# open-rmf/rmf_crowdsim

Measured on AMD Instinct MI355X. Metric: agent-steps/sec at 1M agents, dt=0.05 s; % HBM roofline on Zanlungo kernel, higher is better.
Workload: dtype f32

## Files before the change

### rmf_crowdsim_amd/csrc/crowdstep_hip.hip

```cpp

#include <hip/hip_runtime.h>
#include <chrono>

#include <algorithm>
#include <cmath>
#include <cstdint>
#include <cstdio>
#include <array>
#include <cmath>
#include <cstring>
#include <functional>
#include <map>
#include <string>
#include <thread>
#include <tuple>
#include <vector>

#include "crowdstep.h"
#include "crowdstep_state.h"

#define CS_INVALID_CELL 0xFFFFFFFFu
#define CS_MAX_GROUPS 1048575u
#define CS_SPAWN_OCCUPANCY_RADIUS 0.4
#define CS_ID_LIMIT 0x7FFFFFFFull
// ... 163 lines not shown
      if (const char* w = getenv("CS_FIRST_DEVICE_ID")) {
        const uint64_t d = std::min<uint64_t>((uint64_t)strtoull(w, nullptr, 10), e->id_limit - 2u);
        e->dev_base = e->next_id = (d & ~1ull) | (e->ext_base & 1u);
      }
    }
    const uint32_t nid = (uint32_t)e->next_id;
    if (ok) hipMemcpy(&e->ctr->next_id, &nid, sizeof nid, hipMemcpyHostToDevice);
  }
  if (!ok || e->upload_sinks() != 0 ||
      e->reserve(cfg && cfg->capacity_hint ? cfg->capacity_hint : 1024) != 0) {
    return create_failed(e, "device allocation failed: " + e->error);
  }
  return e;
}

const char* cs_last_error(const cs_engine* e) { return e ? e->error.c_str() : g_create_error.c_str(); }
const char* cs_backend_name(const cs_engine* e) { return e ? e->backend.c_str() : ""; }

uint32_t cs_register_zanlungo(cs_engine* e, const cs_zanlungo_params* p) {
  e->lp_params.push_back(*p);
  e->lp_kinds.push_back(1u);
  e->lp_callbacks.emplace_back();
  return (uint32_t)e->lp_kinds.size() - 1;
}
uint32_t cs_register_no_local_plan(cs_engine* e) {
  cs_zanlungo_params z;
  std::memset(&z, 0, sizeof z);
  z.agent_mass = 1.0;
  z.force_distance = 1.0;
  e->lp_params.push_back(z);
  e->lp_kinds.push_back(0u);
  e->lp_callbacks.emplace_back();
  return (uint32_t)e->lp_kinds.size() - 1;
}
uint32_t cs_register_lp_callback(cs_engine* e, cs_lp_batch_fn fn, void* user) {
  if (!fn) {
    e->error = "cs_register_lp_callback: the planner's function is null";
    return UINT32_MAX;
  }
  cs_zanlungo_params z;
  std::memset(&z, 0, sizeof z);
  z.agent_mass = 1.0;
  z.force_distance = 1.0;
  e->lp_params.push_back(z);
  e->lp_kinds.push_back(2u);
  cs_engine::LpCallback cb;
  cb.fn = fn;
  cb.user = user;
  e->lp_callbacks.push_back(cb);
  return (uint32_t)e->lp_kinds.size() - 1;
}
uint32_t cs_register_hlp(cs_engine* e, const cs_hlp_desc* d) {
  if (d->kind == CS_HLP_ROUTE) {
    if (!d->route_plan || !(d->route_scale > 0.0) || !(d->route_arrive >= 0.0)) {
      e->error = "route planner: route_plan, route_scale > 0 and route_arrive >= 0 are required";
      return UINT32_MAX;
    }
  }
  e->hlps.push_back(*d);
  return (uint32_t)e->hlps.size() - 1;
}

int cs_add_agents(cs_engine* e, const double* xy, size_t n, uint32_t hlp, uint32_t lp,
                  double eyesight, uint64_t* out_ids) {
  hipSetDevice(e->device);
  if (hlp >= e->hlps.size() || lp >= e->lp_kinds.size()) {
    e->error = "unknown planner handle";
    return 2;
  }
  if (e->plain_groups.find(std::make_tuple(hlp, lp, eyesight)) == e->plain_groups.end())
    if (int rc = e->room_for_group(0)) return rc;
  uint32_t g = e->make_group(hlp, lp, eyesight, -1);
  return e->add_agents(xy, n, g, UINT32_MAX, out_ids);
}

int cs_remove_agent(cs_engine* e, uint64_t id) {
  hipSetDevice(e->device);
  e->halo_invalidate();
  for (size_t k = 0; k < e->limbo.size(); ++k)
    if (e->limbo[k].id == id) {
      const HostGroup& g = e->groups[e->limbo[k].group];
      const cs_hlp_desc& p = e->hlps[g.hlp];
      if (p.kind == CS_HLP_CALLBACK && p.remove_agent) p.remove_agent(p.user, id);
      e->limbo.erase(e->limbo.begin() + (long)k);
      cs_event ev;
      ev.kind = CS_EVENT_DESTROYED;
      ev.source_sink = UINT32_MAX;
      ev.id = id;
      ev.x = ev.y = 0;
      if (e->record_events) e->events.push_back(ev);
      return 0;
    }
  if (int rc = e->refresh_counts()) return rc;
  uint32_t found[2] = {0xFFFFFFFFu, 0u};
  uint64_t dev = 0;
  if (e->dev_id(id, &dev) && dev < 0xFFFFFFFFull && e->n_slots) {
    if (!e->find_dev && hipMalloc(&e->find_dev, 2 * sizeof(uint32_t)) != hipSuccess) {
      e->error = "HIP error while removing an agent";
      return 90;
    }
    bool ok = hipMemcpyAsync(e->find_dev, found, sizeof found, hipMemcpyHostToDevice, e->stream) == hipSuccess;
    hipLaunchKernelGGL(k_remove_by_id, dim3((e->n_slots + 255u) / 256u), dim3(256), 0, e->stream, e->gdev, e->buf[e->cur],
                       e->n_slots, e->ctr, e->gdev.tile, (e->tile && e->ghosts_present) ? 1u : 0u, (uint32_t)dev,
                       e->find_dev);
    ok = ok && hipMemcpyAsync(found, e->find_dev, sizeof found, hipMemcpyDeviceToHost, e->stream) == hipSuccess &&
         hipStreamSynchronize(e->stream) == hipSuccess;
    if (!ok) {
      e->error = "HIP error while removing an agent";
      return 90;
    }
  }
  if (found[0] == 0xFFFFFFFFu) {
    e->error = "unknown agent id";
    return 2;
  }
  const HostGroup& g = e->groups[meta_group(e->gdev, found[1])];
  const cs_hlp_desc& p = e->hlps[g.hlp];
  if (p.kind == CS_HLP_CALLBACK && p.remove_agent) p.remove_agent(p.user, id);
  e->sorted = false;
  e->hist_valid = false;
  e->occ_valid = false;
  e->halo_invalidate();
  e->n_alive_host -= 1;
  cs_event ev;
  ev.kind = CS_EVENT_DESTROYED;
  ev.source_sink = g.sink >= 0 ? (uint32_t)g.sink : UINT32_MAX;
  ev.id = id;
  ev.x = ev.y = 0;
  if (e->record_events) e->events.push_back(ev);
  return 0;
}

size_t cs_source_sink_slots(cs_engine* e) { return e->sinks.size(); }
uint64_t cs_device_bytes(cs_engine* e) { return e->device_bytes(); }

uint64_t cs_kernel_stat(cs_engine* e, uint32_t which) {
  hipSetDevice(e->device);
  if (which == CS_STAT_EXCHANGES_AHEAD) return e->n_exchanges_ahead;
  if (which == CS_STAT_EXCHANGES_AHEAD_USED) return e->n_exchanges_ahead_used;
  if (which == CS_STAT_STEPS_ON_KEPT_WINDOWS) return e->n_steps_on_kept_windows;
  if (which == CS_STAT_RENUMBERINGS) return e->n_renumberings;
  if (which == CS_STAT_RENUMBER_NS) return e->renumber_ns;
  if (which == CS_STAT_WINDOWS_LISTED) {
    uint64_t n = 0;
    return e->windows_listed(&n) ? 0 : n;
  }
  Counters c;
  if (e->read_counters(&c)) return 0;
  switch (which) {
    case CS_STAT_WINDOWS_OFF_LDS: return c.n_win_off_lds;
    case CS_STAT_WINDOWS_CHUNKED: return c.n_win_chunked;
#ifdef CS_TILE_TRIPS
    case 100: case 101: case 102: case 103: case 104: case 105: case 106: case 107: case 108: case 109: case 110: case 111:
    case 112: case 113: case 114: case 115: case 116:
      return c.dbg[which - 100];
#endif
    default: return 0;
  }
}

uint32_t cs_add_source_sink(cs_engine* e, const cs_source_sink_desc* d) {
  if (d->n_waypoints == 0) {
    e->error = "a source-sink needs at least one waypoint";
    return UINT32_MAX;
  }
  hipSetDevice(e->device);
  if (e->room_for_group(d->n_waypoints)) return UINT32_MAX;
  HostSink s;
  s.d = *d;
  s.waypoints.assign(d->waypoints_xy, d->waypoints_xy + 2 * d->n_waypoints);
  s.d.waypoints_xy = nullptr;
  uint32_t handle = (uint32_t)e->sinks.size();
  if (e->tile && d->hlp < e->hlps.size() && e->hlps[d->hlp].kind == CS_HLP_ROUTE) {
    s.spawn_route = e->route_lookup(d->hlp, d->source_x, d->source_y, s.waypoints[0], s.waypoints[1]);
    if (!s.spawn_route) {
      e->error = "route planner found no route for this source-sink (tile engines plan at registration)";
      return UINT32_MAX;
    }
  }
  s.group = e->make_group(d->hlp, d->lp, d->agent_eyesight_range, (int32_t)handle);
  e->sinks.push_back(s);
  e->sinks_dirty = true;
  return handle;
}

void cs_remove_source_sink(cs_engine* e, uint32_t handle) {
  if (handle < e->sinks.size() && e->sinks[handle].alive) {
    e->sinks[handle].alive = false;
    e->sinks_dirty = true;
  }
}

int cs_step(cs_engine* e, double dt_seconds, cs_step_report* report) {
  hipSetDevice(e->device);
  const int rc = e->step(dt_seconds, report);
  if (rc == 0) e->steps_done += 1;
  return rc;
}

int cs_snapshot_request(cs_engine* e) {
  hipSetDevice(e->device);
  return e->snapshot_request();
}

int cs_snapshot_acquire(cs_engine* e, int wait, const cs_snapshot_record** out, size_t* n,
                        uint64_t* step_index) {
  hipSetDevice(e->device);
  return e->snapshot_acquire(wait, out, n, step_index);
}

int cs_synchronize(cs_engine* e) {
  hipSetDevice(e->device);
  if (int rc = e->refresh_counts()) return rc;
  Counters c;
  if (int rc = e->read_counters(&c)) return rc;
  e->prof_collect();
  if (c.n_out_of_bounds) {
    e->poisoned = true;
    e->error = "Index out of bounds";
    return 1;
  }
  return 0;
}

size_t cs_agent_count(cs_engine* e) {
  hipSetDevice(e->device);
  e->refresh_counts();
  if (e->tile && e->ghosts_present && e->n_slots) {
    uint32_t owned = 0;
    bool ok = e->find_dev || hipMalloc(&e->find_dev, 2 * sizeof(uint32_t)) == hipSuccess;
    ok = ok && hipMemsetAsync(e->find_dev, 0, sizeof(uint32_t), e->stream) == hipSuccess;
    if (ok)
      hipLaunchKernelGGL(k_tile_count_owned, dim3((e->n_slots + 255u) / 256u), dim3(256), 0, e->stream, e->gdev,
                         e->buf[e->cur], e->n_slots, e->ctr, e->find_dev);
    ok = ok && hipMemcpyAsync(&owned, e->find_dev, sizeof owned, hipMemcpyDeviceToHost, e->stream) == hipSuccess &&
         hipStreamSynchronize(e->stream) == hipSuccess;
    if (ok) return (size_t)owned + e->limbo.size();
    e->error = "HIP error while counting the agents of a tile that holds ghosts";
  }
  return (size_t)e->n_alive_host + e->limbo.size();
}

size_t cs_read_agents(cs_engine* e, cs_agent_view* out, size_t cap) {
  hipSetDevice(e->device);
  if (e->refresh_counts() != 0) return 0;
  cs_engine::HostState h;
  if (e->download(&h) != 0) return 0;
  const bool owned_only = e->tile && e->ghosts_present;
  uint32_t in_use = e->n_slots;
  if (owned_only) {
    Counters c;
    if (e->read_counters(&c) != 0) return 0;
    in_use = std::min(in_use, c.n_pending);
  }
  const GridDev& g = e->gdev;
  std::vector<uint32_t> live;
  for (uint32_t i = 0; i < in_use; ++i) {
    if (h.cell[i] == CS_INVALID_CELL) continue;
    if (owned_only) {
      const uint32_t cx = h.cell[i] / g.nx, cy = h.cell[i] - cx * g.nx;
      if (cx < g.own_x0 || cx >= g.own_x1 || cy < g.own_y0 || cy >= g.own_y1) continue;
    }
    live.push_back(i);
  }
  std::sort(live.begin(), live.end(), [&](uint32_t a, uint32_t b) { return h.id[a] < h.id[b]; });
  size_t n = std::min(cap, live.size());
  for (size_t k = 0; k < n; ++k) {
    uint32_t i = live[k];
    out[k].id = e->ext_id(h.id[i]);
    e->to_global(h.cell[i], h.off[i].x, h.off[i].y, &out[k].x, &out[k].y);
    out[k].vx = h.vel[i].x;
    out[k].vy = h.vel[i].y;
    out[k].next_waypoint = meta_waypoint(e->gdev, h.meta[i]);
    out[k].eyesight_range = e->groups[meta_group(e->gdev, h.meta[i])].eyesight;
  }
  if (!e->limbo.empty()) {
    for (const cs_engine::LimboAgent& l : e->limbo) {
      if (n >= cap) break;
      cs_agent_view v;
      std::memset(&v, 0, sizeof v);
      v.id = l.id;
      v.x = l.x;
      v.y = l.y;
      v.eyesight_range = e->groups[l.group].eyesight;
      out[n++] = v;
    }
    std::sort(out, out + n, [](const cs_agent_view& a, const cs_agent_view& b) { return a.id < b.id; });
  }
  return n;
}

size_t cs_drain_events(cs_engine* e, cs_event* out, size_t cap) {
  size_t n = std::min(cap, e->events.size());
  for (size_t i = 0; i < n; ++i) out[i] = e->events[i];
  e->events.erase(e->events.begin(), e->events.begin() + n);
  return n;
}

void cs_event_recording(cs_engine* e, int on) {
  hipSetDevice(e->device);
  e->refresh_counts();
  e->record_events = on != 0;
  if (!on) e->events.clear();
}

static size_t radius_query(cs_engine* e, double radius, double x, double y, std::vector<uint32_t>* ids,
                           std::vector<float>* d2, size_t cap, bool every_alias) {
// ... 688 lines not shown
```

### rmf_crowdsim_amd/csrc/cs_device_types.hip.inc

```

struct GridDev {
  uint32_t nx;
  uint32_t ny;
  uint32_t ncells;
  float cs;
  float cs_lo;
  float inv_cs;
  uint32_t tile;
  uint32_t own_x0, own_x1, own_y0, own_y1;
  uint32_t org_x, org_y;
  int32_t cs_fix;
  float fix_scale, fix_inv;
  uint32_t grp_bits;
};
__host__ __device__ inline uint32_t meta_group(const GridDev& g, uint32_t meta) { return meta & ((1u << g.grp_bits) - 1u); }
__host__ __device__ inline uint32_t meta_waypoint(const GridDev& g, uint32_t meta) { return meta >> g.grp_bits; }
__host__ __device__ inline uint32_t meta_make(const GridDev& g, uint32_t group, uint32_t waypoint) {
  return group | (waypoint << g.grp_bits);
}

#define FIX_LIM 0x20000000
#define FIX_FAR 0x40000000
__device__ __forceinline__ bool fix_ok(float off, const GridDev& g) {
  return fabsf(off * g.fix_scale) < (float)FIX_LIM;
}
__device__ __forceinline__ int fix_coord(float off, const GridDev& g) {
  return __float2int_rn(off * g.fix_scale);
}
__device__ __forceinline__ void fix_rel(const GridDev& g, float2 oi, float2 oj, int sx, int sy, float& fx,
                                        float& fy) {
  if (fix_ok(oi.x, g) && fix_ok(oi.y, g) && fix_ok(oj.x, g) && fix_ok(oj.y, g) && abs(sx) <= 32 && abs(sy) <= 32) {
    fx = (float)(fix_coord(oj.x, g) - fix_coord(oi.x, g) + sx * g.cs_fix);
    fy = (float)(fix_coord(oj.y, g) - fix_coord(oi.y, g) + sy * g.cs_fix);
  } else {
    fx = ((oj.x + (float)sx * g.cs) - oi.x) * g.fix_scale;
    fy = ((oj.y + (float)sy * g.cs) - oi.y) * g.fix_scale;
  }
}

struct GroupDev {
  float eyesight;
  uint32_t lp_kind;
  float A, D, inv_mass, R;
  uint32_t hlp_kind;
  float hvx, hvy;
  int32_t sink;
  uint32_t hlp;
  float vanish2;
};

struct SelGroupDev {
  uint32_t sink, hlp, lp;
};

struct SinkDev {
  double src_x, src_y;
  uint32_t src_cell;
  uint32_t ghost_cell;
  float src_ox, src_oy;
  float radius_sink;
  uint32_t wp_begin, wp_count;
  uint32_t loop_forever;
  uint32_t group;
  float eyesight;
  uint32_t spawn_route;
};

struct Counters {
  uint32_t n_alive;
  uint32_t n_out_of_bounds;
  uint32_t n_owned;
  uint32_t n_pending;
  uint32_t next_id;
  uint32_t n_spawned;
  uint32_t n_halo_overflow;
  uint32_t n_destroyed;
  uint32_t n_waypoint_hits;
  uint32_t n_tti_zero;
  uint32_t n_nonfinite;
  uint32_t n_clamped;
  uint32_t n_wp_events;
  uint32_t n_halo_late;
  uint32_t n_win_off_lds, n_win_chunked;
  uint32_t n_win_dropped;
  uint32_t n_scan_stalled;
  uint32_t mesh_fail_step;
  uint32_t border_done, border_flag, n_early_stalled;
#ifdef CS_TILE_TRIPS
  uint32_t dbg[17];
#endif
};

struct AgentArrays {
  float2* off;
  float2* vel;
  uint32_t* id;
  uint32_t* cell;
  uint32_t* meta;
  uint32_t* rank;
  uint32_t* route;
};

__device__ __forceinline__ float f_inf() { return __builtin_huge_valf(); }
__device__ __forceinline__ float f_nan() { return __builtin_nanf(""); }

__device__ __forceinline__ float fast_rcp(float x) { return __builtin_amdgcn_rcpf(x); }
__device__ __forceinline__ float fast_sqrt(float x) { return __builtin_amdgcn_sqrtf(x); }
__device__ __forceinline__ float fast_rsq(float x) { return __builtin_amdgcn_rsqf(x); }
__device__ __forceinline__ float fast_exp2(float x) { return __builtin_amdgcn_exp2f(x); }


__device__ __forceinline__ float ttc_select(float t0, float t1) {
  float t = fmaxf(t0, 0.0f);
  t = !(t0 < 0.0f || t0 > 0.0f) ? t1 : t;
  return (t1 > 0.0f) ? t : f_inf();
}

__device__ __noinline__ float ttc_tiny_f32(float rvx, float rvy, float rpx, float rpy, float d2,
                                           float R2, float tscale) {
  rvx *= tscale;
  rvy *= tscale;
  const float a = __builtin_fmaf(rvx, rvx, rvy * rvy);
  const float bh = __builtin_fmaf(rvx, rpx, rvy * rpy);
  const float c = d2 - R2;
  if (a < 1e-30f) {
    if (bh == 0.0f) return f_inf();
    if (c < 0.0f) return 0.0f;
    return bh < 0.0f ? (-c / (2.0f * bh)) * tscale : f_inf();
  }
  const float disc = __builtin_fmaf(bh, bh, -(a * c));
  const float root = fast_sqrt(disc);
  const float ia = fast_rcp(a) * tscale;
  const float t0 = (-bh - root) * ia;
  const float t1 = (-bh + root) * ia;
  return (disc < 0.0f) ? f_inf() : ttc_select(t0, t1);
}

__device__ __forceinline__ float ttc_core_c_f32(float rvx, float rvy, float rpx, float rpy, float c) {
  const float a = __builtin_fmaf(rvx, rvx, rvy * rvy);
  const float bh = __builtin_fmaf(rvx, rpx, rvy * rpy);
  const float disc = __builtin_fmaf(bh, bh, -(a * c));
  const float root = fast_sqrt(disc);
  const float ia = fast_rcp(a);
  const float t0 = (-bh - root) * ia;
  const float t1 = (-bh + root) * ia;
  return ttc_select(t0, t1);
}
__device__ __forceinline__ float ttc_core_f32(float rvx, float rvy, float rpx, float rpy, float d2,
                                              float R2) {
  return ttc_core_c_f32(rvx, rvy, rpx, rpy, d2 - R2);
}

#define TTC_TINY_KEY (0x2B8CBCCCu - 1u)
__device__ __forceinline__ uint32_t ttc_tiny_key(float rvx, float rvy) {
  return __float_as_uint(fmaxf(fabsf(rvx), fabsf(rvy))) - 1u;
}

#define TTC_HUGE_SPEED 0x1p32f
__device__ __forceinline__ bool ttc_huge(float rvx, float rvy) { return fmaxf(fabsf(rvx), fabsf(rvy)) >= TTC_HUGE_SPEED; }

__device__ __forceinline__ float ttc_f32(float rvx, float rvy, float rpx, float rpy, float d2,
                                         float R2) {
  if (__builtin_expect(ttc_tiny_key(rvx, rvy) < TTC_TINY_KEY, 0))
    return ttc_tiny_f32(rvx, rvy, rpx, rpy, d2, R2, 0x1p48f);
  if (__builtin_expect(ttc_huge(rvx, rvy), 0)) return ttc_tiny_f32(rvx, rvy, rpx, rpy, d2, R2, 0x1p-40f);
  return ttc_core_f32(rvx, rvy, rpx, rpy, d2, R2);
}

__device__ __forceinline__ uint32_t ttc_overlap_key(float d2) { return __float_as_uint(d2) - 1u; }
__device__ __forceinline__ float ttc_pair_f32(float rvx, float rvy, float rpx, float rpy, float d2,
                                              float R2) {
  if (__builtin_expect(ttc_overlap_key(d2) < __float_as_uint(R2) || ttc_huge(rvx, rvy), 0))
    return ttc_f32(rvx, rvy, rpx, rpy, d2, R2);
  return ttc_core_c_f32(rvx, rvy, rpx, rpy, d2 - R2);
}

struct ForceCtx {
  float vix, viy, futx, futy, mag, two_R, k_exp;
};

__device__ __forceinline__ ForceCtx make_force_ctx(float vix, float viy, float Ts, const GroupDev& grp, const GridDev& g) {
  ForceCtx c;
  c.vix = vix;
  c.viy = viy;
  c.futx = vix * Ts;
  c.futy = viy * Ts;
  const float T = Ts * g.fix_inv;
  float speed = sqrtf(__builtin_fmaf(vix, vix, viy * viy));
  if (Ts == 0.0f && speed == 0.0f) speed = fmaxf(fabsf(vix), fabsf(viy));
  float mag = 2.0f * grp.A * speed / T;
  c.mag = (mag >= 1e15f) ? 1e15f : mag;
  c.two_R = grp.R * 2.0f * g.fix_scale;
  c.k_exp = 1.44269504088896341f / grp.D * g.fix_inv;
  return c;
}

__device__ __forceinline__ float sight_margin(float ax, float ay, float nr2) {
  return __builtin_fmaf(ax, ax, __builtin_fmaf(ay, ay, nr2));
}

__device__ __forceinline__ bool wave_any(bool p) { return __builtin_amdgcn_ballot_w64(p) != 0ull; }
__device__ __forceinline__ uint32_t in_vgpr(uint32_t x) {
  uint32_t v;
  asm volatile("v_mov_b32 %0, %1" : "=v"(v) : "s"(x));
  return v;
}

#define CS_LDS __attribute__((address_space(3)))
__device__ __forceinline__ uint32_t lds_addr(const void* p) { return (uint32_t)(uintptr_t)(CS_LDS const char*)p; }
typedef int cs_v4i __attribute__((ext_vector_type(4)));
typedef int cs_v2i __attribute__((ext_vector_type(2)));
typedef float cs_v2f __attribute__((ext_vector_type(2)));
__device__ __forceinline__ int4 lds_ld_i4(uint32_t a) {
  const cs_v4i v = *(CS_LDS const cs_v4i*)(uintptr_t)a;
  return make_int4(v.x, v.y, v.z, v.w);
}
__device__ __forceinline__ int2 lds_ld_i2(uint32_t a) {
  const cs_v2i v = *(CS_LDS const cs_v2i*)(uintptr_t)a;
  return make_int2(v.x, v.y);
}
__device__ __forceinline__ float2 lds_ld_f2(uint32_t a) {
  const cs_v2f v = *(CS_LDS const cs_v2f*)(uintptr_t)a;
  return make_float2(v.x, v.y);
}
__device__ __forceinline__ uint32_t lds_ld_u32(uint32_t a) { return *(CS_LDS const uint32_t*)(uintptr_t)a; }
__device__ __forceinline__ uint32_t lds_ld_u16(uint32_t a) { return *(CS_LDS const unsigned short*)(uintptr_t)a; }
__device__ __forceinline__ void lds_st_u16(uint32_t a, uint32_t v) { *(CS_LDS unsigned short*)(uintptr_t)a = (unsigned short)v; }

__device__ __forceinline__ void zanlungo_forward_force(float rpx, float rpy, float d2,
                                                       const ForceCtx& c, float& fx, float& fy) {
  const float dx = c.futx - rpx, dy = c.futy - rpy;
  const float dist = fast_sqrt(__builtin_fmaf(dx, dx, dy * dy));
  float px = rpy, py = -rpx;
  const bool flip = __builtin_fmaf(px, c.vix, py * c.viy) < 0.0f;
  px = flip ? -px : px;
  py = flip ? -py : py;
  const float s = fabsf(__builtin_fmaf(px, dy, -(py * dx)));
  const float inv_n = (s > 0.0f) ? fast_rsq(d2) : f_nan();
  const float scale = c.mag * fast_exp2((c.two_R - dist) * c.k_exp) * inv_n;
  fx = __builtin_fmaf(px, scale, fx);
  fy = __builtin_fmaf(py, scale, fy);
}

#define ZAN_EXP2_ZERO 160.0f

__device__ __forceinline__ bool zanlungo_forward_vanishes(const ForceCtx& c, float Ts, float vanish2) {
  const float fut2 = __builtin_fmaf(c.futx, c.futx, c.futy * c.futy);
  return Ts > 0.0f && Ts < f_inf() && fabsf(c.mag) < f_inf() && fut2 >= vanish2;
}
inline float zanlungo_vanish2(float eyesight, float R, float D, const GridDev& g) {
  const float k_exp = 1.44269504088896341f / D * g.fix_inv;
  const float rs = eyesight * g.fix_scale, two_R = R * 2.0f * g.fix_scale;
  if (!(k_exp >= 0x1p-126f && k_exp < HUGE_VALF && std::fabs(rs) < HUGE_VALF && std::fabs(two_R) < HUGE_VALF))
    return std::nanf("");
  const double b = ((double)std::fabs(rs) + std::max((double)two_R, 0.0) + (double)ZAN_EXP2_ZERO / (double)k_exp) *
                   (1.0 + 0x1p-10);
  const float b2 = std::nextafter((float)(b * b), HUGE_VALF);
  return b2 < HUGE_VALF ? b2 : std::nanf("");
}

struct RouteBookEntry {
  long long sx, sy, gx, gy;
  uint32_t hlp, route1;
};
__host__ __device__ inline long long route_spatial_hash(double v, double res) {
  const double r = round(v / res);
  if (r != r) return 0;
  if (r >= 9.2e18) return 0x7FFFFFFFFFFFFFFFll;
  if (r <= -9.2e18) return (long long)0x8000000000000000ull;
  return (long long)r;
}
__host__ __device__ inline uint32_t route_book_slot(uint32_t hlp, long long sx, long long sy, long long gx, long long gy) {
  unsigned long long h = 0x9E3779B97F4A7C15ull * (unsigned long long)(hlp + 1u);
  h = (h ^ (unsigned long long)sx) * 0xBF58476D1CE4E5B9ull;
  h = (h ^ (unsigned long long)sy) * 0x94D049BB133111EBull;
  h = (h ^ (unsigned long long)gx) * 0xBF58476D1CE4E5B9ull;
  h = (h ^ (unsigned long long)gy) * 0x94D049BB133111EBull;
  return (uint32_t)(h >> 32);
}
__device__ __forceinline__ uint32_t route_book_find(const RouteBookEntry* __restrict__ book, uint32_t mask,
                                                    uint32_t hlp, long long sx, long long sy, long long gx,
                                                    long long gy) {
  if (!book) return 0u;
  uint32_t k = route_book_slot(hlp, sx, sy, gx, gy) & mask;
  for (uint32_t probe = 0; probe <= mask; ++probe) {
    const RouteBookEntry e = book[k];
    if (e.route1 == 0u) return 0u;
    if (e.hlp == hlp && e.sx == sx && e.sy == sy && e.gx == gx && e.gy == gy) return e.route1;
    k = (k + 1u) & mask;
  }
  return 0u;
}

struct StepParams {
  GridDev g;
  float dt;
  uint32_t n;
  uint32_t has_sinks;
  uint32_t n_src_cells;
  uint32_t halo_late_check;
  uint32_t peek_seq;
};

// ... 131 lines not shown
```

### rmf_crowdsim_amd/csrc/cs_kernels_step.hip.inc

```

struct WpEvent {
  uint32_t id, group, next_wp, cell;
  float ox, oy;
  uint32_t slot, pad;
};

struct EpilogueCore {
  AgentArrays out;
  uint32_t* cell_count;
  Counters* ctr;
  const GroupDev* groups;
  const SinkDev* sinks;
  const double* waypoints;
  double grid_off_x, grid_off_y, cell_size;
  uint2* destroyed;
  uint32_t destroyed_cap;
  WpEvent* wp_events;
  uint32_t wp_events_cap;
  const uint32_t* src_cell_start;
  const uint32_t* src_sorted;
  uint32_t* src_occupied;
  const uint2* route_desc;
  const double* route_xy;
  const RouteBookEntry* route_book;
// ... 890 lines not shown
  const bool tile_huge = XF ? (tile_flags & 1u) != 0u : tile_flags != 0u;
  bool lds_ok = tiled_ok;
  if constexpr (XF) {
    if (tiled_ok && (tile_flags & 2u) != 0u) {
      lds_ok = false;
      if (tid == 0) atomicAdd(&E.ctr->n_win_off_lds, 1u);
    }
  }
  for (uint32_t chunk = 0; chunk < n_own; chunk += TILE_THREADS) {
  const OwnIn L = chunk == 0 ? first_own : load_own(chunk);
  const bool active = L.active;
  const int R = row0 + L.own_r;
  const uint32_t i = L.i;
  Own o;
  o.gx = (uint32_t)R;
  o.gy = L.cell - (uint32_t)R * g.nx;
  o.off = L.off;
  o.v = L.v;
  o.id = L.id;
  o.slot = i;
  const uint32_t meta = L.meta;
  const GroupDev grp = L.grp;
  uint32_t route_st = L.route;
  o.u = active ? hlp_velocity(grp, E, g, o.id, pref, i, o.gx, o.gy, o.off, route_st) : make_float2(0.0f, 0.0f);
  float wx = o.u.x, wy = o.u.y;
  if (active && grp.lp_kind == 2u && E.lp_vel) {
    wx = E.lp_vel[i].x;
    wy = E.lp_vel[i].y;
  }
  const bool zan = active && grp.lp_kind == 1u && o.off.x == o.off.x && o.off.y == o.off.y;
  const bool sight_ok = fabsf(grp.eyesight) < f_inf();

  int lx = 1, hx = 0, ly = 1, hy = 0;
  bool use_tile = false;
  if (zan) {
    const float slack = 0.01f * g.cs;
    const bool regular = o.off.x >= -slack && o.off.x <= g.cs + slack && o.off.y >= -slack &&
                         o.off.y <= g.cs + slack;
    if (lds_ok && regular && sight_ok) {
      const float e = grp.eyesight, ics = g.inv_cs;
      const int blx = (int)fminf(fmaxf(floorf((o.off.x - e) * ics - CS_BOUNDS_EPS), -1e9f), 1e9f);
      const int bhx = (int)fminf(fmaxf(floorf((o.off.x + e) * ics + CS_BOUNDS_EPS), -1e9f), 1e9f);
      const int bly = (int)fminf(fmaxf(floorf((o.off.y - e) * ics - CS_BOUNDS_EPS), -1e9f), 1e9f);
      const int bhy = (int)fminf(fmaxf(floorf((o.off.y + e) * ics + CS_BOUNDS_EPS), -1e9f), 1e9f);
      use_tile = (long long)o.gy + bhy < (long long)g.nx;
      lx = max(blx, -cfg.h);
      hx = min(bhx, cfg.h);
      ly = max(bly, -cfg.h);
      hy = min(bhy, cfg.h);
    }
  }
  if (zan && !use_tile) {
    bool tz;
    gather_agent(P, in, cell_start, o, grp, wx, wy, tz);
    if (tz) atomicAdd(&E.ctr->n_tti_zero, 1u);
  }

  if (lds_ok && !TILE_DEBUG(1u)) {
    const bool mine = zan && use_tile;
    if (!mine) {
      lx = 1; hx = 0; ly = 1; hy = 0;
    }
    const float rs = grp.eyesight * g.fix_scale;
    const float nr2 = -(rs * rs);
    const float Rs = grp.R * g.fix_scale;
    const float R2 = Rs * Rs;
    const int own_row = R - r0;
    const int own_col = (int)o.gy - sy0;
    const int2 pi = window_pos(o.off, own_row, own_col);
    const float pix = (float)pi.x;
    auto rel_x = [&](int xj) {
      if constexpr (XF) return __int_as_float(xj) - pix;
      else return (float)(xj - pi.x);
    };
    uint32_t self_slot = 0xFFFFFFFFu;
    if (mine) {
      if (chunk == 0) {
        self_slot = s_self[tid];
      } else {
        const unsigned short* t = s_tab + own_row * W1 + own_col;
        for (uint32_t j = t[0]; j < t[1]; ++j)
          if (s_id[j] == o.id) self_slot = j;
      }
    }
    entry_t* __restrict__ my_list = s_list + tid;
    const uint32_t CAP = cfg.list_cap;
    const uint32_t CAP_ALL = CAP + cfg.spill_rows;
    uint32_t* __restrict__ my_spill =
        cfg.spill + ((size_t)lidx * cfg.spill_rows) * TILE_THREADS + tid;
    bool spilling = false;
    auto entry_at = [&](uint32_t k) -> uint32_t {
      if (k < CAP) return my_list[k * TILE_THREADS];
      return my_spill[(size_t)(k - CAP) * TILE_THREADS];
    };
    uint32_t cnt = 0, n_back = 0;
    unsigned long long fwd = 0;
    unsigned long long fwd2 = 0;
    float T = f_inf();
    bool flushed = false;
    bool self_listed = false;

    auto rel = [&](uint32_t j, float& rpx, float& rpy) {
      const int2 pj = s_pos[j];
      rpx = rel_x(pj.x);
      rpy = (float)(pj.y - pi.y);
    };
    const uint32_t slot_max = S ? S - 1u : 0u;
    auto run_ttc_impl = [&](uint32_t n, uint32_t k0, auto spill_tag) {
      constexpr bool SPILL = decltype(spill_tag)::value;
      uint32_t m_lo = 0, m_hi = 0, m_2 = 0, m_3 = 0;
      for (uint32_t k = k0; __any(k < n); k += 2) {
        const bool v0 = k < n, v1 = k + 1u < n;
        uint32_t j0, j1;
        if (!SPILL || k < CAP) {
          j0 = my_list[k * TILE_THREADS];
          j1 = my_list[(k + 1) * TILE_THREADS];
        } else {
          j0 = v0 ? entry_at(k) : 0u;
          j1 = v1 ? entry_at(k + 1u) : 0u;
        }
        j0 = min(j0, slot_max);
        j1 = min(j1, slot_max);
        const int2 pj0 = s_pos[j0], pj1 = s_pos[j1];
        const float2 vj0 = s_vel[j0], vj1 = s_vel[j1];
        const uint32_t id0 = s_id[j0], id1 = s_id[j1];
        const float rpx0 = rel_x(pj0.x), rpy0 = (float)(pj0.y - pi.y);
        const float rpx1 = rel_x(pj1.x), rpy1 = (float)(pj1.y - pi.y);
        const float rvx0 = vj0.x - o.v.x, rvy0 = vj0.y - o.v.y, rvx1 = vj1.x - o.v.x, rvy1 = vj1.y - o.v.y;
        const float d20 = __builtin_fmaf(rpx0, rpx0, rpy0 * rpy0), d21 = __builtin_fmaf(rpx1, rpx1, rpy1 * rpy1);
        float t0, t1;
        if (tile_huge || __any(min(ttc_overlap_key(d20), ttc_overlap_key(d21)) < __float_as_uint(R2))) {
          t0 = ttc_pair_f32(rvx0, rvy0, rpx0, rpy0, d20, R2);
          t1 = ttc_pair_f32(rvx1, rvy1, rpx1, rpy1, d21, R2);
        } else {
          t0 = ttc_core_f32(rvx0, rvy0, rpx0, rpy0, d20, R2);
          t1 = ttc_core_f32(rvx1, rvy1, rpx1, rpy1, d21, R2);
        }
        t0 = v0 ? t0 : f_inf();
        t1 = v1 ? t1 : f_inf();
        T = fminf(T, fminf(t0, t1));
        const bool f0 = v0 && id0 > o.id, f1 = v1 && id1 > o.id;
        if (k < 32u) m_lo |= (f0 ? (1u << k) : 0u) | (f1 ? (2u << k) : 0u);
        else if (!SPILL || k < 64u) m_hi |= (f0 ? (1u << (k - 32u)) : 0u) | (f1 ? (2u << (k - 32u)) : 0u);
        else if (k < 96u) m_2 |= (f0 ? (1u << (k - 64u)) : 0u) | (f1 ? (2u << (k - 64u)) : 0u);
        else m_3 |= (f0 ? (1u << (k - 96u)) : 0u) | (f1 ? (2u << (k - 96u)) : 0u);
      }
      const unsigned long long m = ((unsigned long long)m_hi << 32) | m_lo;
      const unsigned long long mm = SPILL ? (((unsigned long long)m_3 << 32) | m_2) : 0ull;
      n_back += (n > k0 ? n - k0 : 0u) - (uint32_t)__popcll(m) - (uint32_t)__popcll(mm);
      if (!k0) fwd = 0ull;
      fwd |= m;
      fwd2 = mm;
    };
    auto run_ttc_lds = [&](uint32_t n) {
      if (n & 1u) my_list[n * TILE_THREADS] = my_list[(n - 1u) * TILE_THREADS];
      const float T_in = T;
      uint32_t w0 = 0u, w1 = 0u;
      uint32_t kmin = 0xFFFFFFFFu;
      auto pass = [&](auto guarded_tag) {
        constexpr bool GUARDED = decltype(guarded_tag)::value;
        const entry_t* __restrict__ lp = my_list;
        for (uint32_t kb = 0; kb < 64u; kb += 32u) {
        uint32_t word = 0u, k = kb;
        const uint32_t k_end = min(n, kb + 32u);
        bool v = k < k_end;
        if (wave_any(v)) do {
          if (v) {
            const uint32_t j0 = lp[0], j1 = lp[TILE_THREADS];
            lp += 2 * TILE_THREADS;
            const int2 pj0 = s_pos[j0], pj1 = s_pos[j1];
            const float2 vj0 = s_vel[j0], vj1 = s_vel[j1];
            const uint32_t id0 = s_id[j0], id1 = s_id[j1];
            const float rpx0 = rel_x(pj0.x), rpy0 = (float)(pj0.y - pi.y);
            const float rpx1 = rel_x(pj1.x), rpy1 = (float)(pj1.y - pi.y);
            const float rvx0 = vj0.x - o.v.x, rvy0 = vj0.y - o.v.y, rvx1 = vj1.x - o.v.x, rvy1 = vj1.y - o.v.y;
            const float d20 = __builtin_fmaf(rpx0, rpx0, rpy0 * rpy0), d21 = __builtin_fmaf(rpx1, rpx1, rpy1 * rpy1);
            float t0, t1;
            if (GUARDED) {
              t0 = ttc_pair_f32(rvx0, rvy0, rpx0, rpy0, d20, R2);
              t1 = ttc_pair_f32(rvx1, rvy1, rpx1, rpy1, d21, R2);
            } else {
              kmin = min(kmin, min(ttc_overlap_key(d20), ttc_overlap_key(d21)));
              t0 = ttc_core_f32(rvx0, rvy0, rpx0, rpy0, d20, R2);
              t1 = ttc_core_f32(rvx1, rvy1, rpx1, rpy1, d21, R2);
              word = __builtin_amdgcn_alignbit(word, o.id - id0, 31);
              word = __builtin_amdgcn_alignbit(word, o.id - id1, 31);
            }
            T = fminf(T, fminf(t0, t1));
          }
          k += 2u;
          v = k < k_end;
        } while (wave_any(v));
        if (!GUARDED) {
          w0 = (kb == 0u) ? word : w0;
          w1 = (kb == 0u) ? w1 : word;
        }
        if (!wave_any(kb + 32u < n)) break;
        }
      };
      pass(std::false_type{});
#ifdef CS_TILE_TRIPS
      if ((tid & 63u) == 0u && wave_any(kmin < __float_as_uint(R2))) atomicAdd(&E.ctr->dbg[8], 1u);
#endif
      if (wave_any(kmin < __float_as_uint(R2)) || tile_huge) {
        T = T_in;
        pass(std::true_type{});
      }
      const uint32_t n2 = (n + 1u) & ~1u;
      const uint32_t b0 = min(n2, 32u), b1 = n2 > 32u ? n2 - 32u : 0u;
      uint32_t m_lo = b0 ? __builtin_bitreverse32(w0 << ((32u - b0) & 31u)) : 0u;
      uint32_t m_hi = b1 ? __builtin_bitreverse32(w1 << ((32u - b1) & 31u)) : 0u;
      const unsigned long long valid = n >= 64u ? ~0ull : ((1ull << n) - 1ull);
      const unsigned long long m = ((((unsigned long long)m_hi) << 32) | m_lo) & valid;
      n_back += n - (uint32_t)__popcll(m);
      fwd = m;
      fwd2 = 0ull;
    };
    auto run_ttc = [&](uint32_t n) {
#ifdef CS_TILE_TRIPS
      {
        uint32_t t = 0;
        while (wave_any(2u * t < n)) ++t;
        uint32_t sum = n;
        for (int d = 32; d; d >>= 1) sum += __shfl_xor(sum, d);
        if ((tid & 63u) == 0u) {
          atomicAdd(&E.ctr->dbg[4], t);
          atomicAdd(&E.ctr->dbg[7], sum);
        }
      }
#endif
      if (TILE_DEBUG(32u)) {
        if (!spilling) run_ttc_impl(n, 0u, std::false_type{});
        else run_ttc_impl(n, 0u, std::true_type{});
      } else {
        run_ttc_lds(min(n, CAP));
        if (spilling && wave_any(n > CAP)) run_ttc_impl(n, CAP, std::true_type{});
      }
    };
    float fx = 0.0f, fy = 0.0f;
    ForceCtx fc;
    auto run_force_impl = [&](unsigned long long mask, unsigned long long mask2, auto spill_tag) {
      constexpr bool SPILL = decltype(spill_tag)::value;
      while (mask) {
        const int k = __ffsll((long long)mask) - 1;
        mask &= mask - 1ull;
        float rpx, rpy;
        rel(SPILL ? entry_at((uint32_t)k) : (uint32_t)my_list[k * TILE_THREADS], rpx, rpy);
        const float d2 = __builtin_fmaf(rpx, rpx, rpy * rpy);
        zanlungo_forward_force(rpx, rpy, d2, fc, fx, fy);
      }
      if (SPILL)
        while (mask2) {
          const int k = __ffsll((long long)mask2) - 1;
          mask2 &= mask2 - 1ull;
          float rpx, rpy;
          rel(entry_at(64u + (uint32_t)k), rpx, rpy);
          const float d2 = __builtin_fmaf(rpx, rpx, rpy * rpy);
          zanlungo_forward_force(rpx, rpy, d2, fc, fx, fy);
        }
    };
    auto run_force = [&](unsigned long long mask, unsigned long long mask2) {
#ifdef CS_TILE_TRIPS
      {
        const uint32_t pc = (uint32_t)__popcll(mask) + (uint32_t)__popcll(mask2);
        uint32_t t = 0;
        while (wave_any(t < pc)) ++t;
        uint32_t sum = pc;
        for (int d = 32; d; d >>= 1) sum += __shfl_xor(sum, d);
        if ((tid & 63u) == 0u) {
          atomicAdd(&E.ctr->dbg[3], t);
          atomicAdd(&E.ctr->dbg[6], sum);
        }
      }
#endif
      if (!spilling) {
        run_force_impl(mask, 0ull, std::false_type{});
      } else {
        const unsigned long long in_lds = CAP >= 64u ? ~0ull : ((1ull << CAP) - 1ull);
        run_force_impl(mask & in_lds, 0ull, std::false_type{});
        if (wave_any(((mask & ~in_lds) | mask2) != 0ull)) run_force_impl(mask & ~in_lds, mask2, std::true_type{});
      }
    };
    auto forward_terms_vanish = [&](unsigned long long mask) {
      uint32_t worst = 0u;
      auto word = [&](uint32_t w, uint32_t row0) {
        const entry_t* __restrict__ lp = my_list + row0 * TILE_THREADS;
        while (w) {
          const uint32_t k = (uint32_t)__builtin_ctz(w);
          w &= w - 1u;
          float rpx, rpy;
          rel((uint32_t)lp[k * TILE_THREADS], rpx, rpy);
          const float s = __builtin_fmaf(rpy, fc.futy - rpy, rpx * (fc.futx - rpx));
          worst = max(worst, (__float_as_uint(s) << 1) - 1u);
        }
      };
      word((uint32_t)mask, 0u);
      word((uint32_t)(mask >> 32), 32u);
      return worst <= 0xFEFFFFFFu;
    };
    auto run_force_first = [&](uint32_t c) {
      const unsigned long long lo = c >= 64u ? ~0ull : ((1ull << c) - 1ull);
      const unsigned long long hi = c <= 64u ? 0ull : (c >= 128u ? ~0ull : ((1ull << (c - 64u)) - 1ull));
      run_force(lo, hi);
    };
    auto sweep = [&](bool FORCE) {
      for (int dx = -cfg.h; dx <= cfg.h; ++dx) {
        const int rr = own_row + dx;
        uint32_t j0 = 0, e = 0;
        if (dx >= lx && dx <= hx && rr >= 0 && rr < nr) {
          const int c_lo = max(own_col + ly, 0), c_hi = min(own_col + hy, W1 - 2);
          if (c_lo <= c_hi) {
            j0 = s_tab[rr * W1 + c_lo];
            e = s_tab[rr * W1 + c_hi + 1];
          }
        }
        if (TILE_DEBUG(16u)) j0 = e;
        const uint32_t n_run = e - j0;
        const uint32_t k_first = 0u - (j0 & 1u);
        {
          const uint32_t cnt0 = cnt;
          bool fits;
          if (!FORCE && !TILE_DEBUG(32u)) {
            const uint32_t lbase = lds_addr(my_list), row_bytes = TILE_THREADS * (uint32_t)sizeof(entry_t);
            const uint32_t lim = lbase + CAP * row_bytes;
            const uint32_t far = lds_addr(s_pos + S);
            auto lean_run = [&](auto spill_tag) {
              constexpr bool SPILL = decltype(spill_tag)::value;
              const uint32_t span = cfg.spill_rows * row_bytes;
              uint32_t lp = lbase + cnt * row_bytes;
              uint32_t spilled_to = max(lp, lim);
              uint32_t ja = j0 & ~1u;
              uint32_t src = lds_addr(s_pos + ja);
              bool v = ja < e;
              if (wave_any(v)) do {
#ifdef CS_TILE_TRIPS
                if ((tid & 63u) == 0u) atomicAdd(&E.ctr->dbg[5], 1u);
#endif
                const int4 pp = lds_ld_i4(v ? src : far);
                const float ax = rel_x(pp.x), ay = (float)(pp.y - pi.y);
                const float bx = rel_x(pp.z), by = (float)(pp.w - pi.y);
                const float sa = sight_margin(ax, ay, nr2), sb = sight_margin(bx, by, nr2);
                const uint32_t la = lp;
                lds_st_u16(min(lp, lim), ja);
                lp += (__float_as_uint(sa) >> 22) & row_bytes;
                const uint32_t lb = lp;
                lds_st_u16(min(lp, lim), ja + 1u);
                lp += (__float_as_uint(sb) >> 22) & row_bytes;
                if (SPILL) {
                  const bool late = lp > spilled_to;
                  if (wave_any(late)) {
                    if (late) {
                      if (lb != la && la >= lim && la - lim < span) my_spill[(la - lim) / sizeof(entry_t)] = ja;
                      if (lp != lb && lb >= lim && lb - lim < span) my_spill[(lb - lim) / sizeof(entry_t)] = ja + 1u;
                      spilled_to = lp;
                    }
                  }
                }
                ja += 2u;
                src += 2u * (uint32_t)sizeof(int2);
                v = ja < e;
              } while (wave_any(v));
              cnt = (lp - lbase) / row_bytes;
            };
            fits = true;
            if (!spilling) {
              lean_run(std::false_type{});
              if (dx == 0) self_listed = mine && nr2 < 0.0f;
              if (!wave_any(cnt > CAP)) continue;
              if (cfg.spill_rows) {
                spilling = true;
                cnt = cnt0;
              } else {
                fits = false;
              }
            }
            if (spilling) {
              lean_run(std::true_type{});
              if (dx == 0) self_listed = mine && nr2 < 0.0f;
              fits = !wave_any(cnt > CAP_ALL);
            }
            if (!fits && dx == 0) self_listed = false;
          } else if (!spilling) {
            auto pairs = [&](auto centre_tag) {
              constexpr bool CENTRE = decltype(centre_tag)::value;
              uint32_t k = k_first;
              const int4* __restrict__ src = reinterpret_cast<const int4*>(s_pos + (j0 & ~1u));
              while (__any((int)k < (int)n_run)) {
                const int4 pp = *src;
                const float ax = rel_x(pp.x), ay = (float)(pp.y - pi.y);
                const float bx = rel_x(pp.z), by = (float)(pp.w - pi.y);
                bool ta = sight_margin(ax, ay, nr2) < 0.0f && k < n_run;
                bool tb = sight_margin(bx, by, nr2) < 0.0f && k + 1u < n_run;
                const uint32_t ja = j0 + k;
                if (CENTRE) {
                  ta = ta && ja != self_slot;
                  tb = tb && ja + 1u != self_slot;
                }
                if (FORCE) {
                  if (ta) ta = s_id[ja] > o.id;
                  if (tb) tb = s_id[ja + 1u] > o.id;
                }
                my_list[min(cnt, CAP) * TILE_THREADS] = (entry_t)ja;
                cnt += ta ? 1u : 0u;
                my_list[min(cnt, CAP) * TILE_THREADS] = (entry_t)(ja + 1u);
                cnt += tb ? 1u : 0u;
                k += 2u;
                src += 1;
              }
            };
            if (dx == 0) pairs(std::true_type{});
            else pairs(std::false_type{});
            if (!__any(cnt > CAP)) continue;
            fits = false;
            if (cfg.spill_rows) {
              spilling = true;
              cnt = cnt0;
            }
          }
          if (spilling && (FORCE || TILE_DEBUG(32u))) {
            uint32_t k = k_first;
            const int4* __restrict__ src = reinterpret_cast<const int4*>(s_pos + (j0 & ~1u));
            while (__any((int)k < (int)n_run)) {
              const int4 pp = *src;
              const float ax = rel_x(pp.x), ay = (float)(pp.y - pi.y);
              const float bx = rel_x(pp.z), by = (float)(pp.w - pi.y);
              const uint32_t ja = j0 + k;
              bool ta = sight_margin(ax, ay, nr2) < 0.0f && ja != self_slot && k < n_run;
              bool tb = sight_margin(bx, by, nr2) < 0.0f && ja + 1u != self_slot && k + 1u < n_run;
              if (FORCE) {
                if (ta) ta = s_id[ja] > o.id;
                if (tb) tb = s_id[ja + 1u] > o.id;
              }
              my_list[min(cnt, CAP) * TILE_THREADS] = (entry_t)ja;
              if (ta && cnt >= CAP && cnt < CAP_ALL) my_spill[(size_t)(cnt - CAP) * TILE_THREADS] = ja;
              cnt += ta ? 1u : 0u;
              my_list[min(cnt, CAP) * TILE_THREADS] = (entry_t)(ja + 1u);
              if (tb && cnt >= CAP && cnt < CAP_ALL) my_spill[(size_t)(cnt - CAP) * TILE_THREADS] = ja + 1u;
              cnt += tb ? 1u : 0u;
              k += 2u;
              src += 1;
            }
            fits = !__any(cnt > CAP_ALL);
          }
          if (fits) continue;
          cnt = cnt0;
          if (__any(cnt > CAP)) {
            if (FORCE) {
              run_force_first(cnt);
            } else {
              run_ttc(cnt);
              flushed = true;
            }
            cnt = 0;
          }
        }
        uint32_t j = j0;
        while (__any(j < e)) {
          while (j < e && cnt < CAP) {
            const int2 pj = s_pos[j];
            const float ax = rel_x(pj.x), ay = (float)(pj.y - pi.y);
            bool take = sight_margin(ax, ay, nr2) < 0.0f && j != self_slot;
            if (FORCE && take) take = s_id[j] > o.id;
            if (take) {
              my_list[cnt * TILE_THREADS] = (entry_t)j;
              ++cnt;
            }
            ++j;
          }
          if (__any(cnt >= CAP)) {
            if (FORCE) {
              run_force_first(cnt);
            } else {
              run_ttc(cnt);
              flushed = true;
            }
            cnt = 0;
          }
        }
      }
    };

    PHASE_MARK(6);
    sweep(false);
    PHASE_MARK(7);
#ifdef CS_TILE_TRIPS
    if ((tid & 63u) == 0u) {
      atomicAdd(&E.ctr->dbg[0], 1u);
      if (spilling) atomicAdd(&E.ctr->dbg[1], 1u);
      if (flushed) atomicAdd(&E.ctr->dbg[2], 1u);
    }
#endif
    if (TILE_DEBUG(8u)) cnt = 0;
    run_ttc(cnt);
    PHASE_MARK(8);
    if (self_listed) n_back -= 1u;
    const bool tz = (T == 0.0f);
#ifdef CS_TILE_TRIPS
    {
      const uint32_t n_mine = (uint32_t)__popcll(__ballot(mine)), n_finite = (uint32_t)__popcll(__ballot(mine && T != f_inf()));
      if ((tid & 63u) == 0u) {
        atomicAdd(&E.ctr->dbg[9], n_mine);
        atomicAdd(&E.ctr->dbg[10], n_finite);
      }
    }
#endif
    if (mine && T != f_inf()) fc = make_force_ctx(o.v.x, o.v.y, T, grp, g);
    else fc = ForceCtx{0.f, 0.f, 0.f, 0.f, 0.f, 0.f, 0.f};
    const bool vanish = mine && T != f_inf() && zanlungo_forward_vanishes(fc, T, grp.vanish2);
#ifdef CS_TILE_TRIPS
    {
      const unsigned long long finite = __ballot(mine && T != f_inf()), pass = __ballot(vanish);
      const uint32_t all = (mine && T != f_inf()) ? (uint32_t)__popcll(fwd) + (uint32_t)__popcll(fwd2) : 0u;
      uint32_t ent = vanish ? all : 0u, ent_all = all;
      for (int d = 32; d; d >>= 1) {
        ent += __shfl_xor(ent, d);
        ent_all += __shfl_xor(ent_all, d);
      }
      if ((tid & 63u) == 0u) {
        atomicAdd(&E.ctr->dbg[11], (uint32_t)__popcll(pass));
        if (finite != 0ull && (finite & ~pass) == 0ull) atomicAdd(&E.ctr->dbg[12], 1u);
        atomicAdd(&E.ctr->dbg[13], ent);
        atomicAdd(&E.ctr->dbg[16], ent_all);
      }
    }
#endif
    if (TILE_DEBUG(64u)) {
    } else if (!__any(flushed)) {
      unsigned long long m = (T != f_inf()) ? fwd : 0ull;
      const unsigned long long work = __builtin_amdgcn_ballot_w64(m != 0ull);
      if (!TILE_DEBUG(~0u) && !spilling && work != 0ull && (work & ~__builtin_amdgcn_ballot_w64(vanish)) == 0ull) {
        if (m != 0ull && forward_terms_vanish(m)) m = 0ull;
#ifdef CS_TILE_TRIPS
        {
          const unsigned long long fast = __ballot(vanish && m == 0ull);
          if ((tid & 63u) == 0u) {
            atomicAdd(&E.ctr->dbg[14], (uint32_t)__popcll(fast));
            if (!wave_any(m != 0ull)) atomicAdd(&E.ctr->dbg[15], 1u);
          }
        }
#endif
      }
      run_force(m, (T != f_inf()) ? fwd2 : 0ull);
    } else {
      cnt = 0;
      if (T == f_inf()) {
        lx = 1; hx = 0;
      }
      sweep(true);
      run_force_first(cnt);
    }
    if (mine) {
      if (T != f_inf()) {
        if (tz && n_back > 0) {
          fx = f_nan();
          fy = f_nan();
        }
      } else {
        fx = 0.0f;
        fy = 0.0f;
      }
      wx = __builtin_fmaf(fx, grp.inv_mass, o.u.x);
      wy = __builtin_fmaf(fy, grp.inv_mass, o.u.y);
      if (tz) atomicAdd(&E.ctr->n_tti_zero, 1u);
    }
    PHASE_MARK(9);
  }
  if (active && !TILE_DEBUG(4u)) step_epilogue(P, E, Ep, i, o.gx, o.gy, o.off, o.id, meta, grp, wx, wy, route_st, late_check);
  PHASE_MARK(10);
  }
  BORDER_DONE();
  PHASE_END();
}
#undef BORDER_DONE

__global__ void k_wait_border(Counters* __restrict__ ctr, uint32_t seq) {
  if (threadIdx.x != 0) return;
  for (uint32_t spins = 0; spins < (1u << 22); ++spins) {
    if (__hip_atomic_load(&ctr->border_flag, __ATOMIC_ACQUIRE, __HIP_MEMORY_SCOPE_AGENT) == seq) return;
    __builtin_amdgcn_s_sleep(16);
  }
  atomicAdd(&ctr->n_early_stalled, 1u);
}
```

Before: 7.414 billion.

## Split final TTC pass into cheap skip-key screen plus sparse exact finish

For the final neighbor-list flush, when every lane's velocity equals its preferred velocity, the TTC loop first computes a cheap sign key (discriminant plus |b|) per pair, avoiding the sqrt and reciprocal. It packs which pairs could yield a finite collision time into a bitmask. Only those pairs are then revisited to compute the exact time-to-collision. This removes transcendental work for non-colliding pairs, at the cost of a second divergent gather pass over the surviving pairs, and it only helps when few pairs survive. Debug counters are extended to measure the split path.

```diff
diff --git a/rmf_crowdsim_amd/csrc/crowdstep_hip.hip b/rmf_crowdsim_amd/csrc/crowdstep_hip.hip
--- a/rmf_crowdsim_amd/csrc/crowdstep_hip.hip
+++ b/rmf_crowdsim_amd/csrc/crowdstep_hip.hip
@@ -339,7 +339,7 @@
     case CS_STAT_WINDOWS_CHUNKED: return c.n_win_chunked;
 #ifdef CS_TILE_TRIPS
     case 100: case 101: case 102: case 103: case 104: case 105: case 106: case 107: case 108: case 109: case 110: case 111:
-    case 112: case 113: case 114: case 115: case 116:
+    case 112: case 113: case 114: case 115: case 116: case 117: case 118: case 119:
       return c.dbg[which - 100];
 #endif
     default: return 0;
diff --git a/rmf_crowdsim_amd/csrc/cs_device_types.hip.inc b/rmf_crowdsim_amd/csrc/cs_device_types.hip.inc
--- a/rmf_crowdsim_amd/csrc/cs_device_types.hip.inc
+++ b/rmf_crowdsim_amd/csrc/cs_device_types.hip.inc
@@ -87,7 +87,7 @@
   uint32_t mesh_fail_step;
   uint32_t border_done, border_flag, n_early_stalled;
 #ifdef CS_TILE_TRIPS
-  uint32_t dbg[17];
+  uint32_t dbg[20];
 #endif
 };
 
@@ -149,6 +149,13 @@
 __device__ __forceinline__ float ttc_core_f32(float rvx, float rvy, float rpx, float rpy, float d2,
                                               float R2) {
   return ttc_core_c_f32(rvx, rvy, rpx, rpy, d2 - R2);
+}
+
+__device__ __forceinline__ uint32_t ttc_skip_key(float rvx, float rvy, float rpx, float rpy, float c) {
+  const float a = __builtin_fmaf(rvx, rvx, rvy * rvy);
+  const float bh = __builtin_fmaf(rvx, rpx, rvy * rpy);
+  const float disc = __builtin_fmaf(bh, bh, -(a * c));
+  return __float_as_uint(disc + __builtin_fabsf(bh)) - 1u;
 }
 
 #define TTC_TINY_KEY (0x2B8CBCCCu - 1u)
diff --git a/rmf_crowdsim_amd/csrc/cs_kernels_step.hip.inc b/rmf_crowdsim_amd/csrc/cs_kernels_step.hip.inc
--- a/rmf_crowdsim_amd/csrc/cs_kernels_step.hip.inc
+++ b/rmf_crowdsim_amd/csrc/cs_kernels_step.hip.inc
@@ -1066,16 +1066,20 @@
       fwd |= m;
       fwd2 = mm;
     };
-    auto run_ttc_lds = [&](uint32_t n) {
+    auto run_ttc_lds = [&](uint32_t n, auto may_split_tag) {
+      constexpr bool MAY_SPLIT = decltype(may_split_tag)::value;
       if (n & 1u) my_list[n * TILE_THREADS] = my_list[(n - 1u) * TILE_THREADS];
       const float T_in = T;
+      const bool split = MAY_SPLIT && !wave_any(n != 0u && (o.v.x != o.u.x || o.v.y != o.u.y));
       uint32_t w0 = 0u, w1 = 0u;
+      uint32_t l0 = 0u, l1 = 0u;
       uint32_t kmin = 0xFFFFFFFFu;
-      auto pass = [&](auto guarded_tag) {
-        constexpr bool GUARDED = decltype(guarded_tag)::value;
+      auto pass = [&](auto form_tag) {
+        constexpr int FORM = decltype(form_tag)::value;
+        constexpr bool GUARDED = FORM == 1;
         const entry_t* __restrict__ lp = my_list;
         for (uint32_t kb = 0; kb < 64u; kb += 32u) {
-        uint32_t word = 0u, k = kb;
+        uint32_t word = 0u, lword = 0u, k = kb;
         const uint32_t k_end = min(n, kb + 32u);
         bool v = k < k_end;
         if (wave_any(v)) do {
@@ -1089,18 +1093,23 @@
             const float rpx1 = rel_x(pj1.x), rpy1 = (float)(pj1.y - pi.y);
             const float rvx0 = vj0.x - o.v.x, rvy0 = vj0.y - o.v.y, rvx1 = vj1.x - o.v.x, rvy1 = vj1.y - o.v.y;
             const float d20 = __builtin_fmaf(rpx0, rpx0, rpy0 * rpy0), d21 = __builtin_fmaf(rpx1, rpx1, rpy1 * rpy1);
-            float t0, t1;
             if (GUARDED) {
-              t0 = ttc_pair_f32(rvx0, rvy0, rpx0, rpy0, d20, R2);
-              t1 = ttc_pair_f32(rvx1, rvy1, rpx1, rpy1, d21, R2);
+              const float t0 = ttc_pair_f32(rvx0, rvy0, rpx0, rpy0, d20, R2);
+              const float t1 = ttc_pair_f32(rvx1, rvy1, rpx1, rpy1, d21, R2);
+              T = fminf(T, fminf(t0, t1));
             } else {
               kmin = min(kmin, min(ttc_overlap_key(d20), ttc_overlap_key(d21)));
-              t0 = ttc_core_f32(rvx0, rvy0, rpx0, rpy0, d20, R2);
-              t1 = ttc_core_f32(rvx1, rvy1, rpx1, rpy1, d21, R2);
+              if (FORM == 0) {
+                const float t0 = ttc_core_f32(rvx0, rvy0, rpx0, rpy0, d20, R2);
+                const float t1 = ttc_core_f32(rvx1, rvy1, rpx1, rpy1, d21, R2);
+                T = fminf(T, fminf(t0, t1));
+              } else {
+                lword = __builtin_amdgcn_alignbit(lword, ttc_skip_key(rvx0, rvy0, rpx0, rpy0, d20 - R2), 31);
+                lword = __builtin_amdgcn_alignbit(lword, ttc_skip_key(rvx1, rvy1, rpx1, rpy1, d21 - R2), 31);
+              }
               word = __builtin_amdgcn_alignbit(word, o.id - id0, 31);
               word = __builtin_amdgcn_alignbit(word, o.id - id1, 31);
             }
-            T = fminf(T, fminf(t0, t1));
           }
           k += 2u;
           v = k < k_end;
@@ -1108,29 +1117,72 @@
         if (!GUARDED) {
           w0 = (kb == 0u) ? word : w0;
           w1 = (kb == 0u) ? w1 : word;
+          if (FORM == 2) {
+            l0 = (kb == 0u) ? lword : l0;
+            l1 = (kb == 0u) ? l1 : lword;
+          }
         }
         if (!wave_any(kb + 32u < n)) break;
         }
       };
-      pass(std::false_type{});
+      if constexpr (MAY_SPLIT) {
+        if (split) pass(std::integral_constant<int, 2>{});
+        else pass(std::integral_constant<int, 0>{});
+      } else {
+        pass(std::integral_constant<int, 0>{});
+      }
 #ifdef CS_TILE_TRIPS
+      if ((tid & 63u) == 0u && split) atomicAdd(&E.ctr->dbg[19], 1u);
       if ((tid & 63u) == 0u && wave_any(kmin < __float_as_uint(R2))) atomicAdd(&E.ctr->dbg[8], 1u);
 #endif
+      const uint32_t n2 = (n + 1u) & ~1u;
+      const uint32_t b0 = min(n2, 32u), b1 = n2 > 32u ? n2 - 32u : 0u;
+      const unsigned long long valid = n >= 64u ? ~0ull : ((1ull << n) - 1ull);
       if (wave_any(kmin < __float_as_uint(R2)) || tile_huge) {
         T = T_in;
-        pass(std::true_type{});
-      }
-      const uint32_t n2 = (n + 1u) & ~1u;
-      const uint32_t b0 = min(n2, 32u), b1 = n2 > 32u ? n2 - 32u : 0u;
+        pass(std::integral_constant<int, 1>{});
+      } else if (split) {
+        if constexpr (MAY_SPLIT) {
+          auto finish = [&](uint32_t w, uint32_t row0) {
+            const entry_t* __restrict__ lp = my_list + row0 * TILE_THREADS;
+            while (w) {
+              const uint32_t k = (uint32_t)__builtin_ctz(w);
+              w &= w - 1u;
+              const uint32_t j = lp[k * TILE_THREADS];
+              const float2 vj = s_vel[j];
+              float rpx, rpy;
+              rel(j, rpx, rpy);
+              const float d2 = __builtin_fmaf(rpx, rpx, rpy * rpy);
+              T = fminf(T, ttc_core_f32(vj.x - o.v.x, vj.y - o.v.y, rpx, rpy, d2, R2));
+            }
+          };
+          const uint32_t live_lo = ~__builtin_bitreverse32(l0 << ((32u - b0) & 31u)) & (uint32_t)valid;
+          const uint32_t live_hi = ~__builtin_bitreverse32(l1 << ((32u - b1) & 31u)) & (uint32_t)(valid >> 32);
+#ifdef CS_TILE_TRIPS
+          {
+            const uint32_t pc = (uint32_t)__popc(live_lo) + (uint32_t)__popc(live_hi);
+            uint32_t t = 0;
+            while (wave_any(t < pc)) ++t;
+            uint32_t sum = pc;
+            for (int d = 32; d; d >>= 1) sum += __shfl_xor(sum, d);
+            if ((tid & 63u) == 0u) {
+              atomicAdd(&E.ctr->dbg[17], t);
+              atomicAdd(&E.ctr->dbg[18], sum);
+            }
+          }
+#endif
+          finish(live_lo, 0u);
+          if (wave_any(live_hi != 0u)) finish(live_hi, 32u);
+        }
+      }
       uint32_t m_lo = b0 ? __builtin_bitreverse32(w0 << ((32u - b0) & 31u)) : 0u;
       uint32_t m_hi = b1 ? __builtin_bitreverse32(w1 << ((32u - b1) & 31u)) : 0u;
-      const unsigned long long valid = n >= 64u ? ~0ull : ((1ull << n) - 1ull);
       const unsigned long long m = ((((unsigned long long)m_hi) << 32) | m_lo) & valid;
       n_back += n - (uint32_t)__popcll(m);
       fwd = m;
       fwd2 = 0ull;
     };
-    auto run_ttc = [&](uint32_t n) {
+    auto run_ttc = [&](uint32_t n, auto may_split_tag) {
 #ifdef CS_TILE_TRIPS
       {
         uint32_t t = 0;
@@ -1147,7 +1199,7 @@
         if (!spilling) run_ttc_impl(n, 0u, std::false_type{});
         else run_ttc_impl(n, 0u, std::true_type{});
       } else {
-        run_ttc_lds(min(n, CAP));
+        run_ttc_lds(min(n, CAP), may_split_tag);
         if (spilling && wave_any(n > CAP)) run_ttc_impl(n, CAP, std::true_type{});
       }
     };
@@ -1362,7 +1414,7 @@
             if (FORCE) {
               run_force_first(cnt);
             } else {
-              run_ttc(cnt);
+              run_ttc(cnt, std::false_type{});
               flushed = true;
             }
             cnt = 0;
@@ -1385,7 +1437,7 @@
             if (FORCE) {
               run_force_first(cnt);
             } else {
-              run_ttc(cnt);
+              run_ttc(cnt, std::false_type{});
               flushed = true;
             }
             cnt = 0;
@@ -1405,7 +1457,7 @@
     }
 #endif
     if (TILE_DEBUG(8u)) cnt = 0;
-    run_ttc(cnt);
+    run_ttc(cnt, std::true_type{});
     PHASE_MARK(8);
     if (self_listed) n_back -= 1u;
     const bool tz = (T == 0.0f);
```

After: 7.576 billion, median of 6. +2.2%, better.
